# NilFoundation/crypto3-zk

Hardware: AMD Instinct MI355X
Metric: MSM Mpoints/sec, BLS12-381 G1 Pippenger, 2^20 points per GPU (higher is better)
Workload: dtype u32; 1 GPU; BLS12-381 G1 Pippenger MSM, ONE MSM of 1 x 2^20 random points/scalars, bases resident; points_per_gpu=1048576, parallelism=point-range partition x1 + one all-gather of the 144-B partial sums

## Files before the change

### crypto3-zk_amd/csrc/msm_core.hpp

```cpp
#pragma once
#include <algorithm>
#include <string>
#include <type_traits>
#include <vector>

#ifndef ZK_NOINLINE_MUL2
#define ZK_NOINLINE_MUL2 1
#endif
#include "ctx.hpp"
#include "curve.hpp"
#include "msm_ops.hpp"
#include "msm_recode.hpp"
#include "msm_bucket_acc.hpp"
#include "fu_pair.hpp"
#include "fu_quad.hpp"

namespace {

using namespace zkhip;

constexpr uint32_t MSM_LARGE_BUCKET = 128;
constexpr uint32_t MSM_LARGE_CHUNK = 4096;
#ifndef MSM_G1_THREADS
#define MSM_G1_THREADS 64
// ... 6 lines not shown
#endif

template <uint32_t THREADS>
ZK_D void block_inclusive_scan(uint32_t *scratch) {
    const uint32_t t = threadIdx.x;
    __syncthreads();
    for (uint32_t d = 1; d < THREADS; d <<= 1) {
        uint32_t x = t >= d ? scratch[t - d] : 0;
        __syncthreads();
        scratch[t] += x;
        __syncthreads();
    }
}

__global__ __launch_bounds__(256) void msm_scan_local(const uint32_t *__restrict__ hist, uint32_t count, uint32_t *__restrict__ offs,
                                                      uint32_t *__restrict__ block_sums) {
    __shared__ uint32_t part[256];
    const uint32_t t = threadIdx.x, base = blockIdx.x * 1024 + t * 4;
    uint32_t v[4], s = 0;
#pragma unroll
    for (int k = 0; k < 4; ++k) {
        v[k] = base + k < count ? hist[base + k] : 0;
        s += v[k];
    }
    part[t] = s;
    block_inclusive_scan<256>(part);
    uint32_t run = part[t] - s;
#pragma unroll
    for (int k = 0; k < 4; ++k) {
        if (base + k < count) offs[base + k] = run;
        run += v[k];
    }
    if (t == 255) block_sums[blockIdx.x] = part[255];
}

__global__ __launch_bounds__(1024) void msm_scan_top(uint32_t *__restrict__ block_sums, uint32_t nblocks, uint32_t *__restrict__ total) {
    __shared__ uint32_t part[1024];
    const uint32_t t = threadIdx.x;
    const uint32_t per = (nblocks + 1023) / 1024;
    const uint32_t lo = min(nblocks, t * per), hi = min(nblocks, lo + per);
    uint32_t s = 0;
    for (uint32_t i = lo; i < hi; ++i) s += block_sums[i];
    part[t] = s;
    block_inclusive_scan<1024>(part);
    uint32_t run = part[t] - s;
    for (uint32_t i = lo; i < hi; ++i) {
        uint32_t x = block_sums[i];
        block_sums[i] = run;
        run += x;
    }
    if (t == 1023) *total = part[1023];
}

__global__ __launch_bounds__(256) void msm_scan_add(uint32_t *__restrict__ offs, uint32_t count, const uint32_t *__restrict__ block_sums,
                                                    uint32_t *__restrict__ cursor) {
    const uint32_t base = blockIdx.x * 1024 + threadIdx.x * 4;
    const uint32_t add = block_sums[blockIdx.x];
#pragma unroll
    for (int k = 0; k < 4; ++k) {
        if (base + k < count) {
            uint32_t x = offs[base + k] + add;
            offs[base + k] = x;
            cursor[base + k] = x;
        }
    }
}

__global__ __launch_bounds__(1024) void msm_scan_single(const uint32_t *__restrict__ hist, uint32_t count, uint32_t *__restrict__ offs,
                                                        uint32_t *__restrict__ cursor) {
    __shared__ uint32_t part[1024];
    __shared__ uint32_t carry;
    const uint32_t t = threadIdx.x;
    if (t == 0) carry = 0;
    __syncthreads();
    for (uint32_t base = 0; base < count; base += 1024) {
        const uint32_t v = base + t < count ? hist[base + t] : 0;
        part[t] = v;
        block_inclusive_scan<1024>(part);
        const uint32_t excl = carry + part[t] - v;
        if (base + t < count) {
            offs[base + t] = excl;
            if (cursor != offs) cursor[base + t] = excl;
        }
        __syncthreads();
        if (t == 1023) carry += part[1023];
        __syncthreads();
    }
    if (t == 0) offs[count] = carry;
}
constexpr uint32_t MSM_SCAN_SINGLE_MAX = 1u << 16;

inline int msm_scan(zkhip_ctx *ctx, const char *name, const uint32_t *hist, uint32_t count, uint32_t *offs, uint32_t *bsums) {
    if (count <= MSM_SCAN_SINGLE_MAX) {
        ZK_LAUNCH(ctx, name, msm_scan_single, dim3(1), dim3(1024), 0, hist, count, offs, offs);
        return 0;
    }
    const uint32_t nblk = (count + 1023) / 1024;
    ZK_LAUNCH(ctx, name, msm_scan_local, dim3(nblk), dim3(256), 0, hist, count, offs, bsums);
    ZK_LAUNCH(ctx, name, msm_scan_top, dim3(1), dim3(1024), 0, bsums, nblk, offs + count);
    ZK_LAUNCH(ctx, name, msm_scan_add, dim3(nblk), dim3(256), 0, offs, count, bsums, offs);
    return 0;
}

template <class FR>
__global__ __launch_bounds__(256) void msm_digits_only(const uint32_t *__restrict__ scalars, uint32_t n, MsmWindows win, uint32_t wrank,
                                                       uint32_t wworld, uint32_t *__restrict__ dig) {
    uint32_t i = blockIdx.x * blockDim.x + threadIdx.x;
    if (i >= n) return;
    uint32_t s[8];
    const uint32_t flip = msm_fold_scalar<FR>(scalars + (size_t)i * 8, s) ? 0x80000000u : 0u;
    uint32_t carry = 0, next = wrank, lw = 0;
    for (int w = 0; w < win.W; ++w) {
        uint32_t d = msm_recode(s, win.off(w), win.width(w), carry);
        if ((uint32_t)w != next) continue;
        dig[(size_t)lw * n + i] = d == DIG_NONE ? d : d ^ flip;
        next += wworld;
        ++lw;
    }
}

struct SortGeom {
    uint32_t n;
    uint32_t W;
    uint32_t B;
    uint32_t S;
    uint32_t lowb;
    uint32_t nsuper;
    uint32_t tile;
    uint32_t ntile;
    uint32_t slot0;
    uint32_t tables;
    uint32_t bases_n;
    uint32_t base_off;
};
struct SortBig {
    static constexpr uint32_t TILE = 16384, THREADS = 1024;
};
struct SortSmall {
    static constexpr uint32_t TILE = 4096, THREADS = 256;
};
constexpr uint32_t SORT_MAX_LOW = 10;
constexpr uint32_t SORT_MAX_SUPER = 1024;

ZK_D uint32_t sort_key(const SortGeom &g, uint32_t w, uint32_t d) { return (w % g.S) * g.B + (d & 0x7FFFFFFFu); }
ZK_D uint32_t sort_entry(const SortGeom &g, uint32_t w, uint32_t i, uint32_t d) {
    return ((g.tables ? (g.slot0 + w) * g.bases_n : 0u) + g.base_off + i) | (d & 0x80000000u);
}

template <class SZ>
__global__ __launch_bounds__(SZ::THREADS) void msm_sort_hist(const uint32_t *__restrict__ dig, SortGeom g, uint32_t *__restrict__ bh) {
    constexpr uint32_t SORT_TILE = SZ::TILE, SORT_THREADS = SZ::THREADS;
    extern __shared__ uint32_t lh[];
    const uint32_t tile = blockIdx.x, w = blockIdx.y, t = threadIdx.x;
    for (uint32_t k = t; k < g.nsuper; k += SORT_THREADS) lh[k] = 0;
    __syncthreads();
    const uint32_t lo = tile * SORT_TILE, hi = min(g.n, lo + SORT_TILE);
    for (uint32_t i = lo + t; i < hi; i += SORT_THREADS) {
        uint32_t d = dig[(size_t)w * g.n + i];
        if (d != DIG_NONE) atomicAdd(&lh[sort_key(g, w, d) >> g.lowb], 1u);
    }
    __syncthreads();
    const size_t col = (size_t)w * g.ntile + tile, stride = (size_t)g.W * g.ntile;
    for (uint32_t k = t; k < g.nsuper; k += SORT_THREADS) bh[(size_t)k * stride + col] = lh[k];
}

template <uint32_t SORT_THREADS>
ZK_D uint32_t block_excl_scan(uint32_t *v, uint32_t count, uint32_t *scratch ) {
    const uint32_t t = threadIdx.x, per = (count + SORT_THREADS - 1) / SORT_THREADS;
    const uint32_t lo = min(count, t * per), hi = min(count, lo + per);
    uint32_t s = 0;
    for (uint32_t k = lo; k < hi; ++k) s += v[k];
    scratch[t] = s;
    block_inclusive_scan<SORT_THREADS>(scratch);
    const uint32_t total = scratch[SORT_THREADS - 1];
    uint32_t run = scratch[t] - s;
    for (uint32_t k = lo; k < hi; ++k) {
        uint32_t x = v[k];
        v[k] = run;
        run += x;
    }
    __syncthreads();
    return total;
}

template <class SZ>
__global__ __launch_bounds__(SZ::THREADS) void msm_sort_split(const uint32_t *__restrict__ dig, SortGeom g, const uint32_t *__restrict__ bo,
                                                              uint32_t *__restrict__ tmp_idx, uint16_t *__restrict__ tmp_key) {
    constexpr uint32_t SORT_TILE = SZ::TILE, SORT_THREADS = SZ::THREADS;
    extern __shared__ uint32_t sm[];
    uint32_t *loff = sm;
    uint32_t *cur = loff + g.nsuper + 1;
    uint32_t *gbase = cur + g.nsuper;
    uint32_t *scratch = gbase + g.nsuper;
    uint32_t *sidx = scratch + SORT_THREADS;
    uint32_t *skey = sidx + SORT_TILE;
    const uint32_t tile = blockIdx.x, w = blockIdx.y, t = threadIdx.x;
    const size_t col = (size_t)w * g.ntile + tile, stride = (size_t)g.W * g.ntile;
    for (uint32_t k = t; k < g.nsuper; k += SORT_THREADS) {
        loff[k] = 0;
        gbase[k] = bo[(size_t)k * stride + col];
    }
    __syncthreads();
    const uint32_t lo = tile * SORT_TILE, hi = min(g.n, lo + SORT_TILE);
    for (uint32_t i = lo + t; i < hi; i += SORT_THREADS) {
        uint32_t d = dig[(size_t)w * g.n + i];
        if (d != DIG_NONE) atomicAdd(&loff[sort_key(g, w, d) >> g.lowb], 1u);
    }
    __syncthreads();
    const uint32_t total = block_excl_scan<SORT_THREADS>(loff, g.nsuper, scratch);
    if (t == 0) loff[g.nsuper] = total;
    for (uint32_t k = t; k < g.nsuper; k += SORT_THREADS) cur[k] = loff[k];
    __syncthreads();
    for (uint32_t i = lo + t; i < hi; i += SORT_THREADS) {
        uint32_t d = dig[(size_t)w * g.n + i];
        if (d == DIG_NONE) continue;
        const uint32_t key = sort_key(g, w, d);
        const uint32_t r = atomicAdd(&cur[key >> g.lowb], 1u);
        sidx[r] = sort_entry(g, w, i, d);
        skey[r] = key;
    }
    __syncthreads();
    const uint32_t lmask = (1u << g.lowb) - 1;
    for (uint32_t s = t; s < total; s += SORT_THREADS) {
        const uint32_t key = skey[s], bin = key >> g.lowb, pos = gbase[bin] + (s - loff[bin]);
        tmp_idx[pos] = sidx[s];
        tmp_key[pos] = (uint16_t)(key & lmask);
    }
}

constexpr uint32_t SORT_NLOW_MAX = 1u << SORT_MAX_LOW;

template <uint32_t THREADS>
ZK_D void block_scan_counts(const uint32_t *cnt, uint32_t *excl, uint32_t *scratch) {
    constexpr uint32_t CPT = SORT_NLOW_MAX / THREADS;
    const uint32_t t = threadIdx.x;
    uint32_t s = 0;
#pragma unroll
    for (uint32_t k = 0; k < CPT; ++k) s += cnt[t * CPT + k];
    scratch[t] = s;
    block_inclusive_scan<THREADS>(scratch);
    uint32_t run = scratch[t] - s;
#pragma unroll
    for (uint32_t k = 0; k < CPT; ++k) {
        excl[t * CPT + k] = run;
        run += cnt[t * CPT + k];
    }
    __syncthreads();
}

template <class SZ>
__global__ __launch_bounds__(SZ::THREADS) void msm_sort_final(const uint32_t *__restrict__ tmp_idx, const uint16_t *__restrict__ tmp_key, SortGeom g,
                                                              uint32_t nb, const uint32_t *__restrict__ bo, uint32_t *__restrict__ offs,
                                                              uint32_t *__restrict__ idx) {
    constexpr uint32_t SORT_TILE = SZ::TILE, SORT_THREADS = SZ::THREADS;
    __shared__ uint32_t cnt[SORT_NLOW_MAX], cursor[SORT_NLOW_MAX], loff[SORT_NLOW_MAX], cur[SORT_NLOW_MAX], scratch[SORT_THREADS];
    extern __shared__ uint32_t sm[];
    uint32_t *sidx = sm;
    uint16_t *skey = reinterpret_cast<uint16_t *>(sidx + SORT_TILE);
    const uint32_t grp = blockIdx.x, t = threadIdx.x;
    const size_t stride = (size_t)g.W * g.ntile;
    const uint32_t start = bo[(size_t)grp * stride];
    const uint32_t end = bo[(size_t)(grp + 1) * stride];
    const uint32_t nlow = 1u << g.lowb;
    for (uint32_t k = t; k < SORT_NLOW_MAX; k += SORT_THREADS) cnt[k] = 0;
    __syncthreads();
    for (uint32_t k = start + t; k < end; k += SORT_THREADS) atomicAdd(&cnt[tmp_key[k]], 1u);
    __syncthreads();
    block_scan_counts<SORT_THREADS>(cnt, cursor, scratch);
    for (uint32_t k = t; k < nlow; k += SORT_THREADS) {
        const uint32_t bucket = grp * nlow + k;
        cursor[k] += start;
        if (bucket < nb) offs[bucket] = cursor[k];
    }
    if (grp + 1 == g.nsuper && t == 0) offs[nb] = end;
    __syncthreads();
    for (uint32_t c0 = start; c0 < end; c0 += SORT_TILE) {
        const uint32_t c1 = min(end, c0 + SORT_TILE);
        for (uint32_t k = t; k < SORT_NLOW_MAX; k += SORT_THREADS) cnt[k] = 0;
        __syncthreads();
        for (uint32_t k = c0 + t; k < c1; k += SORT_THREADS) atomicAdd(&cnt[tmp_key[k]], 1u);
        __syncthreads();
        block_scan_counts<SORT_THREADS>(cnt, loff, scratch);
        for (uint32_t k = t; k < SORT_NLOW_MAX; k += SORT_THREADS) cur[k] = loff[k];
        __syncthreads();
        for (uint32_t k = c0 + t; k < c1; k += SORT_THREADS) {
            const uint32_t key = tmp_key[k];
            const uint32_t r = atomicAdd(&cur[key], 1u);
            sidx[r] = tmp_idx[k];
            skey[r] = (uint16_t)key;
        }
        __syncthreads();
        for (uint32_t s = t; s < c1 - c0; s += SORT_THREADS) {
            const uint32_t key = skey[s];
            idx[cursor[key] + (s - loff[key])] = sidx[s];
        }
        __syncthreads();
        for (uint32_t k = t; k < SORT_NLOW_MAX; k += SORT_THREADS) cursor[k] += cnt[k];
        __syncthreads();
    }
}

constexpr uint32_t SIZE_BINS = MSM_LARGE_BUCKET + 2;

ZK_D uint32_t size_bin(uint32_t size, uint32_t large) {
    if (size == 0 || size > large) return SIZE_BINS - 1;
    return size > MSM_LARGE_BUCKET ? 0 : 1 + MSM_LARGE_BUCKET - size;
}

__global__ __launch_bounds__(256) void msm_size_hist(const uint32_t *__restrict__ offs, uint32_t nbuckets, uint32_t nblocks,
                                                     uint32_t large, uint32_t *__restrict__ bh) {
    __shared__ uint32_t lh[SIZE_BINS];
    const uint32_t t = threadIdx.x;
    if (t < SIZE_BINS) lh[t] = 0;
    __syncthreads();
    for (uint32_t g = blockIdx.x * 1024 + t; g < min(nbuckets, (blockIdx.x + 1) * 1024); g += 256)
        atomicAdd(&lh[size_bin(offs[g + 1] - offs[g], large)], 1u);
    __syncthreads();
    if (t < SIZE_BINS) bh[(size_t)t * nblocks + blockIdx.x] = lh[t];
}

__global__ __launch_bounds__(256) void msm_size_scatter(const uint32_t *__restrict__ offs, uint32_t nbuckets, uint32_t nblocks,
                                                        uint32_t large, const uint32_t *__restrict__ bo, uint32_t *__restrict__ order) {
    __shared__ uint32_t cur[SIZE_BINS];
    const uint32_t t = threadIdx.x;
    if (t < SIZE_BINS) cur[t] = bo[(size_t)t * nblocks + blockIdx.x];
    __syncthreads();
    for (uint32_t g = blockIdx.x * 1024 + t; g < min(nbuckets, (blockIdx.x + 1) * 1024); g += 256)
        order[atomicAdd(&cur[size_bin(offs[g + 1] - offs[g], large)], 1u)] = g;
}

__global__ __launch_bounds__(256) void msm_plan_large(const uint32_t *__restrict__ offs, uint32_t nbuckets, uint32_t *__restrict__ plan,
                                                      uint32_t *__restrict__ tasks, uint32_t *__restrict__ large, uint32_t task_cap,
                                                      uint32_t large_cap, uint32_t thresh, uint32_t *__restrict__ status) {
    uint32_t g = blockIdx.x * blockDim.x + threadIdx.x;
    if (g >= nbuckets) return;
    uint32_t lo = offs[g], hi = offs[g + 1], size = hi - lo;
    if (size <= thresh) return;
    uint32_t nt = (size + MSM_LARGE_CHUNK - 1) / MSM_LARGE_CHUNK;
    uint32_t first = atomicAdd(&plan[0], nt);
    uint32_t slot = atomicAdd(&plan[1], 1u);
    if (first + nt > task_cap || slot >= large_cap) {
        atomicOr(status, ZK_STATUS_MSM_PLAN_OVERFLOW);
        return;
    }
    for (uint32_t t = 0; t < nt; ++t) {
        tasks[3 * (first + t)] = g;
        tasks[3 * (first + t) + 1] = lo + t * MSM_LARGE_CHUNK;
        tasks[3 * (first + t) + 2] = min(hi, lo + (t + 1) * MSM_LARGE_CHUNK);
    }
    large[3 * slot] = g;
    large[3 * slot + 1] = first;
    large[3 * slot + 2] = nt;
}

template <class F, int LPB>
__global__ __launch_bounds__(128) void msm_bucket_large(const uint32_t *__restrict__ bases, const uint32_t *__restrict__ idx,
                                                        const uint32_t *__restrict__ plan, const uint32_t *__restrict__ tasks,
                                                        uint32_t *__restrict__ partials) {
    constexpr int NL = FieldOps<F>::WORDS;
    extern __shared__ __attribute__((aligned(16))) uint32_t lds[];
    const uint32_t ntasks = plan[0];
    for (uint32_t task = blockIdx.x; task < ntasks; task += gridDim.x) {
        const uint32_t lo = tasks[3 * task + 1], hi = tasks[3 * task + 2], t = threadIdx.x / LPB;
        XYZZ<F> acc = XYZZ<F>::infinity();
        for (uint32_t k = lo + t; k < hi; k += blockDim.x / LPB) {
            uint32_t e = idx[k];
            Affine<F> p = affine_load<F>(bases + (size_t)(e & 0x7FFFFFFFu) * (2 * NL));
            acc = xyzz_madd(acc, p, (e >> 31) != 0);
        }
        xyzz_store<F>(lds + (size_t)t * (4 * NL), acc);
        __syncthreads();
        for (uint32_t d = blockDim.x / LPB / 2; d >= 1; d >>= 1) {
            if (t < d) {
                acc = xyzz_add(xyzz_load<F>(lds + (size_t)t * (4 * NL)), xyzz_load<F>(lds + (size_t)(t + d) * (4 * NL)));
                xyzz_store<F>(lds + (size_t)t * (4 * NL), acc);
            }
            __syncthreads();
        }
        if (t == 0) xyzz_store<F>(partials + (size_t)task * (4 * NL), acc);
        __syncthreads();
    }
}

template <class F, int LPB>
__global__ __launch_bounds__(64) void msm_large_combine(const uint32_t *__restrict__ plan, const uint32_t *__restrict__ large,
                                                        const uint32_t *__restrict__ partials, uint32_t *__restrict__ buckets) {
    constexpr int NL = FieldOps<F>::WORDS;
    extern __shared__ __attribute__((aligned(16))) uint32_t lds[];
    const uint32_t nlarge = plan[1], t = threadIdx.x / LPB;
    for (uint32_t j = blockIdx.x; j < nlarge; j += gridDim.x) {
        const uint32_t g = large[3 * j], first = large[3 * j + 1], nt = large[3 * j + 2];
        XYZZ<F> acc = XYZZ<F>::infinity();
        for (uint32_t k = t; k < nt; k += 64 / LPB) acc = xyzz_add(acc, xyzz_load<F>(partials + (size_t)(first + k) * (4 * NL)));
        if (nt > 1) {
            xyzz_store<F>(lds + (size_t)t * (4 * NL), acc);
            __syncthreads();
            for (uint32_t d = 32 / LPB; d >= 1; d >>= 1) {
                if (t < d && t + d < nt) {
                    acc = xyzz_add(xyzz_load<F>(lds + (size_t)t * (4 * NL)), xyzz_load<F>(lds + (size_t)(t + d) * (4 * NL)));
                    xyzz_store<F>(lds + (size_t)t * (4 * NL), acc);
                }
                __syncthreads();
            }
        }
        if (t == 0) xyzz_store<F>(buckets + (size_t)g * (4 * NL), acc);
// ... 83 lines not shown
    g.B = B;
    g.log_c = (uint32_t)((lb + 1) / 2);
    g.C = 1u << g.log_c;
    g.R = B >> g.log_c;
    g.run = ctx->opt_msm_fold_run > 0 ? (uint32_t)ctx->opt_msm_fold_run : (B >= (1u << 18) ? 8u : 4u);
    g.run = std::max(1u, std::min(g.run, g.R));
    g.m_row = g.C / g.run;
    g.m_col = g.R / g.run;
    return g;
}

template <class FA, int LA, class FT, int LT>
__global__ __launch_bounds__(MSM_TAIL_THREADS, ZK_TAIL_WAVES) void msm_fold(const uint32_t *__restrict__ buckets, MsmFold g, uint32_t *__restrict__ level2) {
    constexpr int NL = FieldOps<FA>::WORDS;
    constexpr uint32_t SA = MSM_TAIL_THREADS / LA, ST = MSM_TAIL_THREADS / LT, PW = 4 * NL;
    extern __shared__ __attribute__((aligned(16))) uint32_t lds[];
    const uint32_t half_wgs = g.B / (SA * g.run);
    const uint32_t w = blockIdx.x / (2 * half_wgs), k = blockIdx.x % (2 * half_wgs);
    const bool col = k >= half_wgs;
    const uint32_t wg = col ? k - half_wgs : k, s = threadIdx.x / LA;
    const uint32_t m = col ? g.m_col : g.m_row, G = SA / m;
    uint32_t first, stride, slot;
    if (!col) {
        first = (wg * G + s / m) * g.C + s % m;
        stride = m;
        slot = s;
    } else {
        const uint32_t j = s / G, ll = s % G;
        first = j * g.C + wg * G + ll;
        stride = m * g.C;
        slot = ll * m + j;
    }
    {
        const uint32_t *src = buckets + ((size_t)w * g.B + first) * PW;
        XYZZ<FA> acc = xyzz_load<FA>(src);
        for (uint32_t i = 1; i < g.run; ++i) acc = xyzz_add(acc, xyzz_load<FA>(src + (size_t)i * stride * PW));
        xyzz_store<FA>(lds + (size_t)slot * PW, acc);
    }
    __syncthreads();
    const uint32_t t = threadIdx.x / LT;
    for (uint32_t half = m / 2; half >= 1; half >>= 1) {
        const uint32_t adds = G * half;
        for (uint32_t idx = t; idx < adds; idx += ST) {
            uint32_t *p = lds + (size_t)((idx / half) * m + idx % half) * PW;
            xyzz_store<FT>(p, xyzz_add(xyzz_load<FT>(p), xyzz_load<FT>(p + (size_t)half * PW)));
        }
        __syncthreads();
    }
    for (uint32_t i = t; i < G; i += ST) {
        const uint32_t o = wg * G + i;
        if (col || o != 0)
            xyzz_store<FT>(level2 + (((size_t)2 * w + (col ? 0 : 1)) * g.C + (col ? o : o - 1)) * PW, xyzz_load<FT>(lds + (size_t)i * m * PW));
    }
}

template <class F>
ZK_D void xyzz_store_canonical_jacobian(uint32_t *dst, const XYZZ<F> &p) {
    constexpr int CW = FieldOps<F>::CANON_WORDS;
    Jacobian<F> j = xyzz_to_jacobian(p);
    FieldOps<F>::to_canonical(dst, j.X);
    FieldOps<F>::to_canonical(dst + CW, j.Y);
    FieldOps<F>::to_canonical(dst + 2 * CW, j.Z);
}

template <class F, int LPB>
__global__ __launch_bounds__(64) void msm_final_fold(const uint32_t *__restrict__ winsum, uint32_t count, uint32_t shift, uint32_t *const *__restrict__ outs,
                                                     uint32_t *__restrict__ out) {
    constexpr int NL = FieldOps<F>::WORDS;
    if (blockIdx.x >= count || threadIdx.x >= LPB) return;
    XYZZ<F> acc = xyzz_load<F>(winsum + ((size_t)2 * blockIdx.x + 1) * (4 * NL));
    if (!acc.is_inf())
        for (uint32_t i = 0; i < shift; ++i) acc = xyzz_dbl(acc);
    acc = xyzz_add(acc, xyzz_load<F>(winsum + (size_t)2 * blockIdx.x * (4 * NL)));
    xyzz_store_canonical_jacobian<F>(outs ? outs[blockIdx.x] : out, acc);
}

template <class F, int LPB>
__global__ __launch_bounds__(64) void msm_final(const uint32_t *__restrict__ winsum, int W, MsmWindows win, uint32_t *__restrict__ out_jac) {
    constexpr int NL = FieldOps<F>::WORDS;
    if (blockIdx.x != 0 || threadIdx.x >= LPB) return;
    XYZZ<F> acc = XYZZ<F>::infinity();
    for (int w = W - 1; w >= 0; --w) {
        if (!acc.is_inf())
            for (int i = 0; i < win.width(w); ++i) acc = xyzz_dbl(acc);
        acc = xyzz_add(acc, xyzz_load<F>(winsum + (size_t)w * (4 * NL)));
    }
    xyzz_store_canonical_jacobian<F>(out_jac, acc);
}

template <class F>
__global__ __launch_bounds__(256) void bases_to_mont(const uint32_t *__restrict__ canon, const uint8_t *__restrict__ inf, uint32_t n,
                                                     uint32_t *__restrict__ pts) {
    typedef FieldOps<F> O;
    uint32_t i = blockIdx.x * blockDim.x + threadIdx.x;
    if (i >= n) return;
    const uint32_t *c = canon + (size_t)i * (2 * O::CANON_WORDS);
    Affine<F> a;
    if (inf != nullptr && inf[i]) a = Affine<F>::infinity();
    else a = {O::from_canonical(c), O::from_canonical(c + O::CANON_WORDS)};
    affine_store<F>(pts + (size_t)i * (2 * O::WORDS), a);
}

template <class F>
__global__ __launch_bounds__(256) void bases_from_mont(const uint32_t *__restrict__ pts, uint32_t n, uint32_t *__restrict__ out,
                                                       uint8_t *__restrict__ inf) {
    typedef FieldOps<F> O;
// ... 215 lines not shown
}

template <class Lane, class Final>
int msm_tail(zkhip_ctx *ctx, const uint32_t *sets, size_t nsets, uint32_t B, uint32_t *segsum, size_t segsum_blocks, uint32_t *winsum, Final final) {
    typedef typename Lane::type TX;
    constexpr int XL = Lane::LANES;
    const MsmTailGeom t = msm_tail_geom<Lane>(ctx, B, nsets);
    if (nsets * t.nblk > segsum_blocks) {
        ctx->last_error = "MSM tail of " + std::to_string(nsets * t.nblk) + " workgroups over a partial-sum buffer for " + std::to_string(segsum_blocks);
        return ZKHIP_ERR_RANGE;
    }
    ZK_MAX_LDS(ctx, (msm_bucket_red<TX, XL>), t.lds_red);
    ZK_LAUNCH(ctx, "msm_bucket_red", (msm_bucket_red<TX, XL>), dim3((unsigned)(nsets * t.nblk)), dim3(MSM_TAIL_THREADS), t.lds_red, sets, B, t.L, t.nseg, t.nblk,
              segsum);
    ZK_LAUNCH(ctx, "msm_window_sum", (msm_window_sum<TX, XL>), dim3((unsigned)nsets), dim3(t.wthreads), t.lds_win, segsum, t.nblk, winsum);
    return final();
}

template <class F>
bool msm_fold_applies(const zkhip_ctx *ctx, uint32_t B, bool tables) {
    if (FieldOps<F>::WORDS > 16 && !ctx->opt_msm_tail_fold_g2) return false;
    if (!tables || ctx->opt_msm_tail_fold <= 0 || B < (1u << std::min(ctx->opt_msm_tail_fold, 30))) return false;
    const MsmFold g = msm_fold_geom(ctx, B);
    const uint32_t sa = MSM_TAIL_THREADS / BucketLane<F>::LANES;
    return g.m_col >= 1 && g.m_row <= sa && g.m_col <= sa && B >= sa * g.run && g.m_row * g.run == g.C && g.m_col * g.run == g.R;
}
template <class F>
struct MsmFoldBuffers {
    static constexpr size_t PW = (size_t)4 * FieldOps<F>::WORDS;
    MsmFold g{};
    size_t nsets = 0;
    uint32_t *level2 = nullptr, *segsum = nullptr, *winsum = nullptr;
    MsmFoldBuffers() = default;
    MsmFoldBuffers(const zkhip_ctx *ctx, uint32_t B, size_t nsets_) : g(msm_fold_geom(ctx, B)), nsets(nsets_) {}
    size_t level2_words() const { return nsets * 2 * g.C * PW; }
    size_t segsum_blocks() const { return nsets * 2 * ((g.C + 63) / 64); }
    template <class Arena>
    void layout(Arena &a) {
        a.take(level2, level2_words());
        a.take(segsum, segsum_blocks() * PW);
        a.take(winsum, nsets * 2 * PW);
    }
};

template <class F, class Lane>
int msm_fold_tail(zkhip_ctx *ctx, const uint32_t *sets, const MsmFoldBuffers<F> &fb, uint32_t *const *d_outs, uint32_t *d_out) {
    constexpr int NL = FieldOps<F>::WORDS;
    typedef typename BucketLane<F>::type FL;
    constexpr int LPB = BucketLane<F>::LANES;
    typedef typename QuadLane<F>::type TQ;
    constexpr int QL = QuadLane<F>::LANES;
    const MsmFold &g = fb.g;
    const size_t nsets = fb.nsets;
    ZK_HIP_CHECK(ctx, hipMemsetAsync(fb.level2, 0, fb.level2_words() * 4, ctx->stream));
    const size_t lds = (size_t)MSM_TAIL_THREADS / LPB * 4 * NL * 4;
    ZK_MAX_LDS(ctx, (msm_fold<FL, LPB, TQ, QL>), lds);
    ZK_LAUNCH(ctx, "msm_fold", (msm_fold<FL, LPB, TQ, QL>), dim3((unsigned)(nsets * (g.B / (MSM_TAIL_THREADS / LPB * g.run)) * 2)), dim3(MSM_TAIL_THREADS), lds,
              sets, g, fb.level2);
    auto level2 = [&](auto lane) -> int {
        typedef decltype(lane) X;
        return msm_tail<X>(ctx, fb.level2, 2 * nsets, g.C, fb.segsum, fb.segsum_blocks(), fb.winsum, [&]() -> int {
            ZK_LAUNCH(ctx, "msm_final", (msm_final_fold<typename X::type, X::LANES>), dim3((unsigned)nsets), dim3(64), 0, fb.winsum, (uint32_t)nsets, g.log_c, d_outs, d_out);
            return 0;
        });
    };
    if (QuadLane<F>::AVAILABLE && ctx->opt_msm_tail_quads && 2 * nsets * g.C <= ((size_t)1 << 18)) return level2(QuadLane<F>());
    return level2(Lane());
}

struct MsmPlan {
    int c, W_all, W;
    uint32_t B, S, nb;
    MsmWindows win;
    uint32_t wrank, wworld;
    bool tables;
};

inline MsmPlan msm_plan(const zkhip_ctx *ctx, const zkhip_bases *bases, size_t n) {
    MsmPlan p;
    p.tables = bases->tables();
    int c = p.tables ? bases->c_tab : ctx->opt_msm_window_bits;
    if (c <= 0) c = zk_msm_auto_window(n);
    p.c = std::max(2, std::min(ZK_MSM_MAX_C, c));
    if (!p.tables) p.c = std::min(p.c, 16);
    p.W_all = msm_windows(zk_scalar_bits(bases->curve), p.c);
    p.win = msm_make_windows(zk_scalar_bits(bases->curve), p.W_all);
    p.wrank = p.tables ? (uint32_t)bases->win_rank : 0u;
    p.wworld = p.tables ? (uint32_t)bases->win_world : 1u;
    p.W = p.tables ? bases->local_windows() : p.W_all;
    p.B = 1u << (p.c - 1);
    if (!p.tables) p.S = (uint32_t)p.W;
    else {
        int s = ctx->opt_msm_sets;
        if (s <= 0) s = (int)((zk_msm_target_lanes() + p.B - 1) / p.B);
        p.S = (uint32_t)std::max(1, std::min(p.W, s));
        while (p.S > 1 && (uint64_t)p.S * p.B > ((uint64_t)SORT_MAX_SUPER << SORT_MAX_LOW)) --p.S;
    }
    p.nb = p.S * p.B;
    return p;
}

template <class SZ>
int msm_sort_run(zkhip_ctx *ctx, const SortGeom &g, uint32_t nbh, const uint32_t *dig, uint32_t *bh, uint32_t *bo, uint32_t *bsums, uint32_t *tmp_idx,
                 uint16_t *tmp_key, uint32_t *offs, uint32_t *idx) {
    const size_t lds_hist = (size_t)g.nsuper * 4;
    const size_t lds_split = ((size_t)3 * g.nsuper + 1 + SZ::THREADS + 2 * SZ::TILE) * 4;
    const size_t lds_final = (size_t)SZ::TILE * 6;
    if (lds_split > 48 * 1024) ZK_MAX_LDS(ctx, msm_sort_split<SZ>, 160 * 1024 - 256);
    if (lds_final > 40 * 1024) ZK_MAX_LDS(ctx, msm_sort_final<SZ>, 160 * 1024 - (4 * SORT_NLOW_MAX + SZ::THREADS) * 4 - 256);
    ZK_LAUNCH(ctx, "msm_sort_hist", msm_sort_hist<SZ>, dim3(g.ntile, g.W), dim3(SZ::THREADS), lds_hist, dig, g, bh);
    ZK_TRY(msm_scan(ctx, "msm_scan", bh, nbh, bo, bsums));
    ZK_LAUNCH(ctx, "msm_sort_split", msm_sort_split<SZ>, dim3(g.ntile, g.W), dim3(SZ::THREADS), lds_split, dig, g, bo, tmp_idx, tmp_key);
    ZK_LAUNCH(ctx, "msm_sort_final", msm_sort_final<SZ>, dim3(g.nsuper), dim3(SZ::THREADS), lds_final, tmp_idx, tmp_key, g, g.S * g.B, bo, offs, idx);
    return 0;
}

struct MsmCall {
    MsmPlan P;
    SortGeom g;
    bool big_tiles;
    uint32_t nbh;
    uint32_t sblk, nsh;
    int Sr;
    uint32_t segsum_blocks;
    bool fold;
    uint32_t large_thresh, large_cap, task_cap;
    size_t entries() const { return (size_t)P.W * g.n; }
};

template <class F>
int msm_call_plan(const zkhip_ctx *ctx, const zkhip_bases *bases, size_t offset, size_t n, bool batch_member, MsmCall &c, std::string &error) {
    const MsmPlan &P = c.P = msm_plan(ctx, bases, n);
    if ((uint64_t)P.W * n >= (1ull << 32) || (uint64_t)bases->nslots * bases->n >= (1ull << 31)) {
        error = "MSM of " + std::to_string(n) + " points x " + std::to_string(P.W) + " windows exceeds the 32-bit entry index (split the range)";
        return ZKHIP_ERR_RANGE;
    }
    SortGeom &g = c.g;
    g.n = (uint32_t)n;
    g.W = (uint32_t)P.W;
    g.B = P.B;
    g.S = P.S;
    g.lowb = (uint32_t)std::min<int>(SORT_MAX_LOW, P.c - 1);
    g.nsuper = (P.nb + (1u << g.lowb) - 1) >> g.lowb;
    c.big_tiles = ctx->opt_msm_sort_tile_log >= 14;
    g.tile = c.big_tiles ? SortBig::TILE : SortSmall::TILE;
    g.ntile = (uint32_t)((n + g.tile - 1) / g.tile);
    g.tables = P.tables ? 1u : 0u;
    g.slot0 = P.tables ? (uint32_t)bases->slot_of_local(0) : 0u;
    g.bases_n = (uint32_t)bases->n;
    g.base_off = (uint32_t)offset;
    if (g.nsuper > SORT_MAX_SUPER) return ZKHIP_ERR_RANGE;
    const size_t nbh64 = (size_t)g.nsuper * g.W * g.ntile;
    if (nbh64 >= (1ull << 31)) return ZKHIP_ERR_RANGE;
    c.nbh = (uint32_t)nbh64;
    c.sblk = (P.nb + 1023) / 1024;
    c.nsh = SIZE_BINS * c.sblk;
    c.Sr = P.tables ? 1 : P.W;
    c.segsum_blocks = std::max(msm_tail_geom<TailLane<F>>(ctx, P.B, c.Sr).nblk, msm_tail_geom<QuadLane<F>>(ctx, P.B, c.Sr).nblk);
    c.fold = !batch_member && msm_fold_applies<F>(ctx, P.B, P.tables);
    c.large_thresh = (uint32_t)std::max<size_t>(MSM_LARGE_BUCKET, 4 * ((c.entries() + P.nb - 1) / P.nb));
    c.large_cap = (uint32_t)(c.entries() / c.large_thresh + 1);
    c.task_cap = (uint32_t)(c.entries() / MSM_LARGE_CHUNK + c.large_cap + 1);
    return 0;
}

template <class F>
struct MsmBuffers {
    static constexpr size_t PW = (size_t)4 * FieldOps<F>::WORDS;
    const MsmCall &c;
    uint32_t *dig, *bh, *bo, *bsums, *tmp_idx;
    uint16_t *tmp_key;
    uint32_t *offs, *idx, *buckets;
    uint32_t *sh, *so, *ssums, *order;
    uint32_t *segsum, *winsum;
    MsmFoldBuffers<F> fb;
    uint32_t *plan, *tasks, *large, *partials;
    MsmBuffers(const zkhip_ctx *ctx, const MsmCall &call) : c(call) {
        if (c.fold) fb = MsmFoldBuffers<F>(ctx, c.P.B, 1);
    }
    template <class Arena>
    void layout(Arena &a) {
        a.take(dig, c.entries());
        a.take(bh, c.nbh);
        a.take(bo, (size_t)c.nbh + 1);
        a.take(bsums, (c.nbh + 1023) / 1024);
        a.take(tmp_idx, c.entries());
        a.take(tmp_key, c.entries());
        a.take(offs, (size_t)c.P.nb + 1);
        a.take(idx, c.entries());
        a.take(buckets, c.P.nb * PW);
        a.take(sh, (size_t)c.nsh + 1);
        a.take(so, (size_t)c.nsh + 1);
        a.take(ssums, (c.nsh + 1023) / 1024);
        a.take(order, c.P.nb);
        a.take(segsum, (size_t)c.Sr * c.segsum_blocks * PW);
        a.take(winsum, (size_t)std::max(1, c.Sr) * PW);
        if (c.fold) fb.layout(a);
        a.take(plan, 4);
        a.take(tasks, (size_t)c.task_cap * 3);
        a.take(large, (size_t)c.large_cap * 3);
        a.take(partials, c.task_cap * PW);
    }
};

template <class F>
int msm_stages(zkhip_ctx *ctx, const zkhip_bases *bases, const MsmCall &c, const MsmBuffers<F> &w, const uint32_t *d_scalars, bool reuse_sort) {
    constexpr int NL = FieldOps<F>::WORDS;
    typedef typename BucketLane<F>::type FL;
    constexpr int LPB = BucketLane<F>::LANES;
    const MsmPlan &P = c.P;
    const uint32_t n = c.g.n, nb = P.nb;
    const uint32_t *d_b = bases->d;
    if (!reuse_sort) {
        unsigned gn = (unsigned)((n + 255) / 256);
        if (bases->curve == CURVE_BLS12_381)
            ZK_LAUNCH(ctx, "msm_digits", msm_digits_only<BlsFr>, dim3(gn), dim3(256), 0, d_scalars, n, P.win, P.wrank, P.wworld, w.dig);
        else ZK_LAUNCH(ctx, "msm_digits", msm_digits_only<BnFr>, dim3(gn), dim3(256), 0, d_scalars, n, P.win, P.wrank, P.wworld, w.dig);
        ZK_TRY((c.big_tiles ? msm_sort_run<SortBig> : msm_sort_run<SortSmall>)(ctx, c.g, c.nbh, w.dig, w.bh, w.bo, w.bsums, w.tmp_idx, w.tmp_key, w.offs, w.idx));
        ZK_LAUNCH(ctx, "msm_size_sort", msm_size_hist, dim3(c.sblk), dim3(256), 0, w.offs, nb, c.sblk, c.large_thresh, w.sh);
        ZK_TRY(msm_scan(ctx, "msm_size_sort", w.sh, c.nsh, w.so, w.ssums));
        ZK_LAUNCH(ctx, "msm_size_sort", msm_size_scatter, dim3(c.sblk), dim3(256), 0, w.offs, nb, c.sblk, c.large_thresh, w.so, w.order);
    }
    if constexpr (FieldOps<F>::WORDS <= 16) {
        constexpr int NT = MSM_G1_THREADS;
        size_t lds_acc = LdsAcc<F, NT>::BYTES;
        ZK_MAX_LDS(ctx, (msm_bucket_acc_lds<F, NT, 3>), lds_acc);
        ZK_LAUNCH(ctx, "msm_bucket_acc", (msm_bucket_acc_lds<F, NT, 3>), dim3((nb + NT - 1) / NT), dim3(NT), lds_acc, d_b, w.offs, w.idx, nb, c.large_thresh,
                  w.order, w.buckets);
    } else {
        constexpr int NT = MSM_G2_THREADS, WAVES = MSM_G2_WAVES;
        size_t lds_acc = LdsAcc<FL, NT>::BYTES;
        ZK_MAX_LDS(ctx, (msm_bucket_acc_lds<FL, NT, WAVES, LPB>), lds_acc);
        ZK_LAUNCH(ctx, "msm_bucket_acc", (msm_bucket_acc_lds<FL, NT, WAVES, LPB>), dim3((unsigned)(((size_t)nb * LPB + NT - 1) / NT)), dim3(NT), lds_acc, d_b,
                  w.offs, w.idx, nb, c.large_thresh, w.order, w.buckets);
    }
    if (!reuse_sort) {
        ZK_HIP_CHECK(ctx, hipMemsetAsync(w.plan, 0, 16, ctx->stream));
        ZK_LAUNCH(ctx, "msm_plan_large", msm_plan_large, dim3((nb + 255) / 256), dim3(256), 0, w.offs, nb, w.plan, w.tasks, w.large, c.task_cap, c.large_cap,
                  c.large_thresh, ctx->d_status);
    }
    {
        size_t lds_large = (size_t)128 / LPB * 4 * NL * 4;
        if (lds_large > 48 * 1024) ZK_MAX_LDS(ctx, (msm_bucket_large<FL, LPB>), lds_large);
        unsigned grid_large = (unsigned)std::min<size_t>(c.task_cap, 512);
        ZK_LAUNCH(ctx, "msm_bucket_large", (msm_bucket_large<FL, LPB>), dim3(grid_large), dim3(128), lds_large, d_b, w.idx, w.plan, w.tasks, w.partials);
        ZK_LAUNCH(ctx, "msm_bucket_large", (msm_large_combine<FL, LPB>), dim3((unsigned)std::min<uint32_t>(c.large_cap, 256)), dim3(64),
                  (size_t)64 / LPB * 4 * NL * 4, w.plan, w.large, w.partials, w.buckets);
    }
    if (P.tables) {
        for (uint32_t cur = P.S; cur > 1;) {
            const uint32_t q = (cur + 3) / 4;
            ZK_LAUNCH(ctx, "msm_bucket_merge", (msm_bucket_merge<FL, LPB>), dim3((unsigned)(((size_t)q * P.B * LPB + 255) / 256)), dim3(256), 0, w.buckets, P.B, q,
                      cur);
            cur = q;
        }
    }
    return 0;
}

template <class F>
int msm_run_t(zkhip_ctx *ctx, const zkhip_bases *bases, size_t offset, size_t n, const uint32_t *d_scalars, uint32_t *d_out_jac) {
    MsmCall c;
    ZK_TRY(msm_call_plan<F>(ctx, bases, offset, n, false, c, ctx->last_error));
    MsmBuffers<F> w(ctx, c);
    ZK_TRY(ws_place(ctx, w));
    ZK_TRY(msm_stages<F>(ctx, bases, c, w, d_scalars, false));
    if (c.fold) return msm_fold_tail<F, TailLane<F>>(ctx, w.buckets, w.fb, nullptr, d_out_jac);
    auto tail = [&](auto lane) -> int {
        typedef decltype(lane) X;
        return msm_tail<X>(ctx, w.buckets, (size_t)c.Sr, c.P.B, w.segsum, (size_t)c.Sr * c.segsum_blocks, w.winsum, [&]() -> int {
            ZK_LAUNCH(ctx, "msm_final", (msm_final<typename X::type, X::LANES>), dim3(1), dim3(64), 0, w.winsum, c.Sr, c.P.win, d_out_jac);
            return 0;
        });
    };
    if (QuadLane<F>::AVAILABLE && ctx->opt_msm_tail_quads && (size_t)c.Sr * c.P.B <= ((size_t)1 << 18)) return tail(QuadLane<F>());
    return tail(TailLane<F>());
}

template <class F>
int msm_batch_member(zkhip_ctx *ctx, const zkhip_bases *bases, size_t offset, size_t n, const uint32_t *d_scalars, uint32_t *slot, bool reuse_sort) {
    MsmCall c;
    ZK_TRY(msm_call_plan<F>(ctx, bases, offset, n, true, c, ctx->last_error));
    MsmBuffers<F> w(ctx, c);
    ZK_TRY(ws_place(ctx, w));
    if (c.P.S == 1) w.buckets = slot;
    ZK_TRY(msm_stages<F>(ctx, bases, c, w, d_scalars, reuse_sort));
    if (w.buckets != slot) ZK_HIP_CHECK(ctx, hipMemcpyAsync(slot, w.buckets, c.P.B * MsmBuffers<F>::PW * 4, hipMemcpyDeviceToDevice, ctx->stream));
    return 0;
}

struct BasesTmp {
    size_t words;
// ... 167 lines not shown
```

Measured before the change: 404.7 Mpoints/s.

## Fuse bucket size histogram and large-bucket planning into sort final, drop launches

Computes the per-bucket size histogram and the large-bucket task plan inside msm_sort_final, which already holds the bucket counts. This removes the separate size_hist and plan_large kernels and a memset; the plan counters are now zeroed in sort_hist. Small scans fold the top-level scan into scan_add, with each block summing its preceding block sums itself. The fold's level2 memset is replaced by writing infinity to the unused slots. The aim is fewer launches and passes over offs, at the cost of extra atomics in sort_final and quadratic redundant summation in scan_add.

```diff
diff --git a/crypto3-zk_amd/csrc/msm_core.hpp b/crypto3-zk_amd/csrc/msm_core.hpp
--- a/crypto3-zk_amd/csrc/msm_core.hpp
+++ b/crypto3-zk_amd/csrc/msm_core.hpp
@@ -82,10 +82,23 @@
     if (t == 1023) *total = part[1023];
 }
 
+constexpr uint32_t MSM_SCAN_SELF_MAX = 1024;
+template <bool SELF>
 __global__ __launch_bounds__(256) void msm_scan_add(uint32_t *__restrict__ offs, uint32_t count, const uint32_t *__restrict__ block_sums,
                                                     uint32_t *__restrict__ cursor) {
     const uint32_t base = blockIdx.x * 1024 + threadIdx.x * 4;
-    const uint32_t add = block_sums[blockIdx.x];
+    uint32_t add;
+    if constexpr (SELF) {
+        __shared__ uint32_t part[256];
+        uint32_t s = 0;
+        for (uint32_t j = threadIdx.x; j < blockIdx.x; j += 256) s += block_sums[j];
+        part[threadIdx.x] = s;
+        block_inclusive_scan<256>(part);
+        add = part[255];
+        if (blockIdx.x + 1 == gridDim.x && threadIdx.x == 0) offs[count] = add + block_sums[blockIdx.x];
+    } else {
+        add = block_sums[blockIdx.x];
+    }
 #pragma unroll
     for (int k = 0; k < 4; ++k) {
         if (base + k < count) {
@@ -127,8 +140,12 @@
     }
     const uint32_t nblk = (count + 1023) / 1024;
     ZK_LAUNCH(ctx, name, msm_scan_local, dim3(nblk), dim3(256), 0, hist, count, offs, bsums);
+    if (nblk <= MSM_SCAN_SELF_MAX) {
+        ZK_LAUNCH(ctx, name, msm_scan_add<true>, dim3(nblk), dim3(256), 0, offs, count, bsums, offs);
+        return 0;
+    }
     ZK_LAUNCH(ctx, name, msm_scan_top, dim3(1), dim3(1024), 0, bsums, nblk, offs + count);
-    ZK_LAUNCH(ctx, name, msm_scan_add, dim3(nblk), dim3(256), 0, offs, count, bsums, offs);
+    ZK_LAUNCH(ctx, name, msm_scan_add<false>, dim3(nblk), dim3(256), 0, offs, count, bsums, offs);
     return 0;
 }
 
@@ -178,10 +195,12 @@
 }
 
 template <class SZ>
-__global__ __launch_bounds__(SZ::THREADS) void msm_sort_hist(const uint32_t *__restrict__ dig, SortGeom g, uint32_t *__restrict__ bh) {
+__global__ __launch_bounds__(SZ::THREADS) void msm_sort_hist(const uint32_t *__restrict__ dig, SortGeom g, uint32_t *__restrict__ bh,
+                                                             uint32_t *__restrict__ plan) {
     constexpr uint32_t SORT_TILE = SZ::TILE, SORT_THREADS = SZ::THREADS;
     extern __shared__ uint32_t lh[];
     const uint32_t tile = blockIdx.x, w = blockIdx.y, t = threadIdx.x;
+    if (tile == 0 && w == 0 && t < 4) plan[t] = 0;
     for (uint32_t k = t; k < g.nsuper; k += SORT_THREADS) lh[k] = 0;
     __syncthreads();
     const uint32_t lo = tile * SORT_TILE, hi = min(g.n, lo + SORT_TILE);
@@ -258,6 +277,45 @@
     }
 }
 
+constexpr uint32_t SIZE_BINS = MSM_LARGE_BUCKET + 2;
+
+ZK_D uint32_t size_bin(uint32_t size, uint32_t large) {
+    if (size == 0 || size > large) return SIZE_BINS - 1;
+    return size > MSM_LARGE_BUCKET ? 0 : 1 + MSM_LARGE_BUCKET - size;
+}
+
+__global__ __launch_bounds__(256) void msm_size_scatter(const uint32_t *__restrict__ offs, uint32_t nbuckets, uint32_t nblocks, uint32_t blk,
+                                                        uint32_t large, const uint32_t *__restrict__ bo, uint32_t *__restrict__ order) {
+    __shared__ uint32_t cur[SIZE_BINS];
+    const uint32_t t = threadIdx.x;
+    if (t < SIZE_BINS) cur[t] = bo[(size_t)t * nblocks + blockIdx.x];
+    __syncthreads();
+    for (uint32_t g = blockIdx.x * blk + t; g < min(nbuckets, (blockIdx.x + 1) * blk); g += 256)
+        order[atomicAdd(&cur[size_bin(offs[g + 1] - offs[g], large)], 1u)] = g;
+}
+
+struct LargePlan {
+    uint32_t *plan, *tasks, *large, *status;
+    uint32_t task_cap, large_cap, thresh;
+};
+ZK_D void msm_plan_large_bucket(const LargePlan &lp, uint32_t g, uint32_t lo, uint32_t hi) {
+    uint32_t nt = (hi - lo + MSM_LARGE_CHUNK - 1) / MSM_LARGE_CHUNK;
+    uint32_t first = atomicAdd(&lp.plan[0], nt);
+    uint32_t slot = atomicAdd(&lp.plan[1], 1u);
+    if (first + nt > lp.task_cap || slot >= lp.large_cap) {
+        atomicOr(lp.status, ZK_STATUS_MSM_PLAN_OVERFLOW);
+        return;
+    }
+    for (uint32_t t = 0; t < nt; ++t) {
+        lp.tasks[3 * (first + t)] = g;
+        lp.tasks[3 * (first + t) + 1] = lo + t * MSM_LARGE_CHUNK;
+        lp.tasks[3 * (first + t) + 2] = min(hi, lo + (t + 1) * MSM_LARGE_CHUNK);
+    }
+    lp.large[3 * slot] = g;
+    lp.large[3 * slot + 1] = first;
+    lp.large[3 * slot + 2] = nt;
+}
+
 constexpr uint32_t SORT_NLOW_MAX = 1u << SORT_MAX_LOW;
 
 template <uint32_t THREADS>
@@ -281,8 +339,9 @@
 template <class SZ>
 __global__ __launch_bounds__(SZ::THREADS) void msm_sort_final(const uint32_t *__restrict__ tmp_idx, const uint16_t *__restrict__ tmp_key, SortGeom g,
                                                               uint32_t nb, const uint32_t *__restrict__ bo, uint32_t *__restrict__ offs,
-                                                              uint32_t *__restrict__ idx) {
+                                                              uint32_t *__restrict__ idx, uint32_t *__restrict__ sh, LargePlan lp) {
     constexpr uint32_t SORT_TILE = SZ::TILE, SORT_THREADS = SZ::THREADS;
+    static_assert(SIZE_BINS <= SORT_THREADS, "the size histogram lives in the scan's scratch words");
     __shared__ uint32_t cnt[SORT_NLOW_MAX], cursor[SORT_NLOW_MAX], loff[SORT_NLOW_MAX], cur[SORT_NLOW_MAX], scratch[SORT_THREADS];
     extern __shared__ uint32_t sm[];
     uint32_t *sidx = sm;
@@ -297,13 +356,20 @@
     for (uint32_t k = start + t; k < end; k += SORT_THREADS) atomicAdd(&cnt[tmp_key[k]], 1u);
     __syncthreads();
     block_scan_counts<SORT_THREADS>(cnt, cursor, scratch);
+    if (t < SIZE_BINS) scratch[t] = 0;
+    __syncthreads();
     for (uint32_t k = t; k < nlow; k += SORT_THREADS) {
         const uint32_t bucket = grp * nlow + k;
         cursor[k] += start;
-        if (bucket < nb) offs[bucket] = cursor[k];
+        if (bucket < nb) {
+            offs[bucket] = cursor[k];
+            atomicAdd(&scratch[size_bin(cnt[k], lp.thresh)], 1u);
+            if (cnt[k] > lp.thresh) msm_plan_large_bucket(lp, bucket, cursor[k], cursor[k] + cnt[k]);
+        }
     }
     if (grp + 1 == g.nsuper && t == 0) offs[nb] = end;
     __syncthreads();
+    if (t < SIZE_BINS) sh[(size_t)t * g.nsuper + grp] = scratch[t];
     for (uint32_t c0 = start; c0 < end; c0 += SORT_TILE) {
         const uint32_t c1 = min(end, c0 + SORT_TILE);
         for (uint32_t k = t; k < SORT_NLOW_MAX; k += SORT_THREADS) cnt[k] = 0;
@@ -328,59 +394,6 @@
         for (uint32_t k = t; k < SORT_NLOW_MAX; k += SORT_THREADS) cursor[k] += cnt[k];
         __syncthreads();
     }
-}
-
-constexpr uint32_t SIZE_BINS = MSM_LARGE_BUCKET + 2;
-
-ZK_D uint32_t size_bin(uint32_t size, uint32_t large) {
-    if (size == 0 || size > large) return SIZE_BINS - 1;
-    return size > MSM_LARGE_BUCKET ? 0 : 1 + MSM_LARGE_BUCKET - size;
-}
-
-__global__ __launch_bounds__(256) void msm_size_hist(const uint32_t *__restrict__ offs, uint32_t nbuckets, uint32_t nblocks,
-                                                     uint32_t large, uint32_t *__restrict__ bh) {
-    __shared__ uint32_t lh[SIZE_BINS];
-    const uint32_t t = threadIdx.x;
-    if (t < SIZE_BINS) lh[t] = 0;
-    __syncthreads();
-    for (uint32_t g = blockIdx.x * 1024 + t; g < min(nbuckets, (blockIdx.x + 1) * 1024); g += 256)
-        atomicAdd(&lh[size_bin(offs[g + 1] - offs[g], large)], 1u);
-    __syncthreads();
-    if (t < SIZE_BINS) bh[(size_t)t * nblocks + blockIdx.x] = lh[t];
-}
-
-__global__ __launch_bounds__(256) void msm_size_scatter(const uint32_t *__restrict__ offs, uint32_t nbuckets, uint32_t nblocks,
-                                                        uint32_t large, const uint32_t *__restrict__ bo, uint32_t *__restrict__ order) {
-    __shared__ uint32_t cur[SIZE_BINS];
-    const uint32_t t = threadIdx.x;
-    if (t < SIZE_BINS) cur[t] = bo[(size_t)t * nblocks + blockIdx.x];
-    __syncthreads();
-    for (uint32_t g = blockIdx.x * 1024 + t; g < min(nbuckets, (blockIdx.x + 1) * 1024); g += 256)
-        order[atomicAdd(&cur[size_bin(offs[g + 1] - offs[g], large)], 1u)] = g;
-}
-
-__global__ __launch_bounds__(256) void msm_plan_large(const uint32_t *__restrict__ offs, uint32_t nbuckets, uint32_t *__restrict__ plan,
-                                                      uint32_t *__restrict__ tasks, uint32_t *__restrict__ large, uint32_t task_cap,
-                                                      uint32_t large_cap, uint32_t thresh, uint32_t *__restrict__ status) {
-    uint32_t g = blockIdx.x * blockDim.x + threadIdx.x;
-    if (g >= nbuckets) return;
-    uint32_t lo = offs[g], hi = offs[g + 1], size = hi - lo;
-    if (size <= thresh) return;
-    uint32_t nt = (size + MSM_LARGE_CHUNK - 1) / MSM_LARGE_CHUNK;
-    uint32_t first = atomicAdd(&plan[0], nt);
-    uint32_t slot = atomicAdd(&plan[1], 1u);
-    if (first + nt > task_cap || slot >= large_cap) {
-        atomicOr(status, ZK_STATUS_MSM_PLAN_OVERFLOW);
-        return;
-    }
-    for (uint32_t t = 0; t < nt; ++t) {
-        tasks[3 * (first + t)] = g;
-        tasks[3 * (first + t) + 1] = lo + t * MSM_LARGE_CHUNK;
-        tasks[3 * (first + t) + 2] = min(hi, lo + (t + 1) * MSM_LARGE_CHUNK);
-    }
-    large[3 * slot] = g;
-    large[3 * slot + 1] = first;
-    large[3 * slot + 2] = nt;
 }
 
 template <class F, int LPB>
@@ -570,6 +583,8 @@
         if (col || o != 0)
             xyzz_store<FT>(level2 + (((size_t)2 * w + (col ? 0 : 1)) * g.C + (col ? o : o - 1)) * PW, xyzz_load<FT>(lds + (size_t)i * m * PW));
     }
+    if (k == 0)
+        for (uint32_t i = g.R - 1 + t; i < g.C; i += ST) xyzz_store<FT>(level2 + (((size_t)2 * w + 1) * g.C + i) * PW, XYZZ<FT>::infinity());
 }
 
 template <class F>
@@ -891,7 +906,6 @@
     constexpr int QL = QuadLane<F>::LANES;
     const MsmFold &g = fb.g;
     const size_t nsets = fb.nsets;
-    ZK_HIP_CHECK(ctx, hipMemsetAsync(fb.level2, 0, fb.level2_words() * 4, ctx->stream));
     const size_t lds = (size_t)MSM_TAIL_THREADS / LPB * 4 * NL * 4;
     ZK_MAX_LDS(ctx, (msm_fold<FL, LPB, TQ, QL>), lds);
     ZK_LAUNCH(ctx, "msm_fold", (msm_fold<FL, LPB, TQ, QL>), dim3((unsigned)(nsets * (g.B / (MSM_TAIL_THREADS / LPB * g.run)) * 2)), dim3(MSM_TAIL_THREADS), lds,
@@ -941,16 +955,16 @@
 
 template <class SZ>
 int msm_sort_run(zkhip_ctx *ctx, const SortGeom &g, uint32_t nbh, const uint32_t *dig, uint32_t *bh, uint32_t *bo, uint32_t *bsums, uint32_t *tmp_idx,
-                 uint16_t *tmp_key, uint32_t *offs, uint32_t *idx) {
+                 uint16_t *tmp_key, uint32_t *offs, uint32_t *idx, uint32_t *sh, const LargePlan &lp) {
     const size_t lds_hist = (size_t)g.nsuper * 4;
     const size_t lds_split = ((size_t)3 * g.nsuper + 1 + SZ::THREADS + 2 * SZ::TILE) * 4;
     const size_t lds_final = (size_t)SZ::TILE * 6;
     if (lds_split > 48 * 1024) ZK_MAX_LDS(ctx, msm_sort_split<SZ>, 160 * 1024 - 256);
     if (lds_final > 40 * 1024) ZK_MAX_LDS(ctx, msm_sort_final<SZ>, 160 * 1024 - (4 * SORT_NLOW_MAX + SZ::THREADS) * 4 - 256);
-    ZK_LAUNCH(ctx, "msm_sort_hist", msm_sort_hist<SZ>, dim3(g.ntile, g.W), dim3(SZ::THREADS), lds_hist, dig, g, bh);
+    ZK_LAUNCH(ctx, "msm_sort_hist", msm_sort_hist<SZ>, dim3(g.ntile, g.W), dim3(SZ::THREADS), lds_hist, dig, g, bh, lp.plan);
     ZK_TRY(msm_scan(ctx, "msm_scan", bh, nbh, bo, bsums));
     ZK_LAUNCH(ctx, "msm_sort_split", msm_sort_split<SZ>, dim3(g.ntile, g.W), dim3(SZ::THREADS), lds_split, dig, g, bo, tmp_idx, tmp_key);
-    ZK_LAUNCH(ctx, "msm_sort_final", msm_sort_final<SZ>, dim3(g.nsuper), dim3(SZ::THREADS), lds_final, tmp_idx, tmp_key, g, g.S * g.B, bo, offs, idx);
+    ZK_LAUNCH(ctx, "msm_sort_final", msm_sort_final<SZ>, dim3(g.nsuper), dim3(SZ::THREADS), lds_final, tmp_idx, tmp_key, g, g.S * g.B, bo, offs, idx, sh, lp);
     return 0;
 }
 
@@ -992,7 +1006,7 @@
     const size_t nbh64 = (size_t)g.nsuper * g.W * g.ntile;
     if (nbh64 >= (1ull << 31)) return ZKHIP_ERR_RANGE;
     c.nbh = (uint32_t)nbh64;
-    c.sblk = (P.nb + 1023) / 1024;
+    c.sblk = g.nsuper;
     c.nsh = SIZE_BINS * c.sblk;
     c.Sr = P.tables ? 1 : P.W;
     c.segsum_blocks = std::max(msm_tail_geom<TailLane<F>>(ctx, P.B, c.Sr).nblk, msm_tail_geom<QuadLane<F>>(ctx, P.B, c.Sr).nblk);
@@ -1051,14 +1065,15 @@
     const uint32_t n = c.g.n, nb = P.nb;
     const uint32_t *d_b = bases->d;
     if (!reuse_sort) {
+        const LargePlan lp = {w.plan, w.tasks, w.large, ctx->d_status, c.task_cap, c.large_cap, c.large_thresh};
         unsigned gn = (unsigned)((n + 255) / 256);
         if (bases->curve == CURVE_BLS12_381)
             ZK_LAUNCH(ctx, "msm_digits", msm_digits_only<BlsFr>, dim3(gn), dim3(256), 0, d_scalars, n, P.win, P.wrank, P.wworld, w.dig);
         else ZK_LAUNCH(ctx, "msm_digits", msm_digits_only<BnFr>, dim3(gn), dim3(256), 0, d_scalars, n, P.win, P.wrank, P.wworld, w.dig);
-        ZK_TRY((c.big_tiles ? msm_sort_run<SortBig> : msm_sort_run<SortSmall>)(ctx, c.g, c.nbh, w.dig, w.bh, w.bo, w.bsums, w.tmp_idx, w.tmp_key, w.offs, w.idx));
-        ZK_LAUNCH(ctx, "msm_size_sort", msm_size_hist, dim3(c.sblk), dim3(256), 0, w.offs, nb, c.sblk, c.large_thresh, w.sh);
+        ZK_TRY((c.big_tiles ? msm_sort_run<SortBig> : msm_sort_run<SortSmall>)(ctx, c.g, c.nbh, w.dig, w.bh, w.bo, w.bsums, w.tmp_idx, w.tmp_key, w.offs, w.idx, w.sh,
+                                                                               lp));
         ZK_TRY(msm_scan(ctx, "msm_size_sort", w.sh, c.nsh, w.so, w.ssums));
-        ZK_LAUNCH(ctx, "msm_size_sort", msm_size_scatter, dim3(c.sblk), dim3(256), 0, w.offs, nb, c.sblk, c.large_thresh, w.so, w.order);
+        ZK_LAUNCH(ctx, "msm_size_sort", msm_size_scatter, dim3(c.sblk), dim3(256), 0, w.offs, nb, c.sblk, 1u << c.g.lowb, c.large_thresh, w.so, w.order);
     }
     if constexpr (FieldOps<F>::WORDS <= 16) {
         constexpr int NT = MSM_G1_THREADS;
@@ -1072,11 +1087,6 @@
         ZK_MAX_LDS(ctx, (msm_bucket_acc_lds<FL, NT, WAVES, LPB>), lds_acc);
         ZK_LAUNCH(ctx, "msm_bucket_acc", (msm_bucket_acc_lds<FL, NT, WAVES, LPB>), dim3((unsigned)(((size_t)nb * LPB + NT - 1) / NT)), dim3(NT), lds_acc, d_b,
                   w.offs, w.idx, nb, c.large_thresh, w.order, w.buckets);
-    }
-    if (!reuse_sort) {
-        ZK_HIP_CHECK(ctx, hipMemsetAsync(w.plan, 0, 16, ctx->stream));
-        ZK_LAUNCH(ctx, "msm_plan_large", msm_plan_large, dim3((nb + 255) / 256), dim3(256), 0, w.offs, nb, w.plan, w.tasks, w.large, c.task_cap, c.large_cap,
-                  c.large_thresh, ctx->d_status);
     }
     {
         size_t lds_large = (size_t)128 / LPB * 4 * NL * 4;
```

After: 401.7 Mpoints/s. Within noise of the previous version (-0.7%).
